# morriscb/chomp

Hardware: AMD Instinct MI355X
Metric: halo-model P(k,z) samples/sec (Stage K set-up + Stage E grid) (higher is better)
Workload: dtype f64

## Files before the change

### chomp_amd/csrc/chomp_mass_kernels.h

```cpp
#pragma once

#include <type_traits>

#include <hip/hip_runtime.h>

#include "../../include/chomp_mi355x.h"
#include "chomp_math.h"
#include "chomp_romberg.h"

namespace chomp {

enum { F_HM = 0, F_PPMM = 1, F_HG = 2, F_PPGM = 3, F_PPGG = 4, F_I12 = 5 };
constexpr int kFamilies = 6;

struct TabLayout {
  int NM, NK;
  int off_ln_mass, off_nu, off_nu_pp, off_lnm_pp;
  int off_knot[6], off_kpp[6];
  int off_levels, off_hf_lns2, off_misc;
  int stride;
  unsigned long long* h_status;
  unsigned h_seq;
};

inline TabLayout make_layout(int NM, int NK) {
  TabLayout L;
  L.NM = NM;
  L.NK = NK;
  int o = 0;
  L.off_ln_mass = o; o += NM;
  L.off_nu = o; o += NM;
  L.off_nu_pp = o; o += 4 * (NM - 1);
  L.off_lnm_pp = o; o += 4 * (NM - 1);
  for (int f = 0; f < kFamilies; ++f) { L.off_knot[f] = o; o += NK; }
  for (int f = 0; f < kFamilies; ++f) { L.off_kpp[f] = o; o += 4 * (NK - 1); }
  L.off_levels = o; o += kFamilies * NK;
  L.off_hf_lns2 = o; o += NK;
  L.off_misc = o; o += 8;
  L.stride = (o + 7) & ~7;
  L.h_status = nullptr;
  L.h_seq = 0u;
  return L;
}

constexpr int kNodeLevel = 10;
constexpr int kNodeTabLevel = 11;
constexpr int kNodeBase = (1 << kNodeLevel) + 1;
constexpr int kNodeCount = (1 << kNodeTabLevel) + 1;
constexpr int kNodeFields = 9;
constexpr int kNodeStride = kNodeFields * kNodeCount + 8;
__host__ __device__ inline int node_index(int lev, long j) {
  return lev == 0 ? (int)j : 1 + (1 << (lev - 1)) + (int)j;
}
typedef const double __attribute__((address_space(1)))* UniformDoubles;
__device__ __forceinline__ UniformDoubles uniform_ptr(const double* p) {
  const unsigned long long v = (unsigned long long)p;
  const unsigned lo = __builtin_amdgcn_readfirstlane((unsigned)v);
  const unsigned hi = __builtin_amdgcn_readfirstlane((unsigned)(v >> 32));
  return (UniformDoubles)(((unsigned long long)hi << 32) | lo);
}

constexpr int kKnotScratch = romberg_scratch<4, 2>();
constexpr int kSearchJ = 2048;
constexpr int kEpochDoubles = (int)(sizeof(Epoch) / sizeof(double));
static_assert(sizeof(Epoch) % sizeof(double) == 0, "Epoch must be 8-byte granular");

__device__ __forceinline__ bool same_cosmology(const Epoch& a, const Epoch& b) {
  return a.om0 == b.om0 && a.ob0 == b.ob0 && a.ol0 == b.ol0 && a.or0 == b.or0 &&
         a.tcmb == b.tcmb && a.h == b.h && a.ns == b.ns;
}

constexpr unsigned kStMassMinSaturated = CHOMP_ST_MASS_MIN_SATURATED;
constexpr unsigned kStMassMaxSaturated = CHOMP_ST_MASS_MAX_SATURATED;
constexpr unsigned kStSearchExhausted = CHOMP_ST_MASS_SEARCH_EXHAUSTED;
constexpr unsigned kStSigmaDivmax = CHOMP_ST_SIGMA_DIVMAX;
constexpr unsigned kStHaloDivmax0 = CHOMP_ST_HALO_DIVMAX_H_M;
constexpr unsigned kStNonfinite = CHOMP_ST_NONFINITE;
constexpr unsigned kStHaloBits = (63u * CHOMP_ST_HALO_DIVMAX_H_M) | CHOMP_ST_NONFINITE;

__device__ __forceinline__ void copy_doubles(double* dst, const double* src, int n) {
  for (int i = threadIdx.x; i < n; i += blockDim.x) dst[i] = src[i];
}

constexpr int kSigmaLevel = 13;
constexpr int kSigmaCount = (1 << kSigmaLevel) + 1;
constexpr int kSGrid = 48;
struct SGrid {
  double b0, b1, b2, b3, b4;
  bool valid;
  __host__ __device__ void segment(double x, double* lo, double* hi, int* n, int* off) const {
    if (x <= b1) { *lo = b0; *hi = b1; *n = 8; *off = 0; }
    else if (x <= b2) { *lo = b1; *hi = b2; *n = 14; *off = 8; }
    else if (x <= b3) { *lo = b2; *hi = b3; *n = 18; *off = 22; }
    else { *lo = b3; *hi = b4; *n = 8; *off = 40; }
  }
  __host__ __device__ double ln_r(int i) const {
    double lo, hi;
    int n, off;
    if (i < 8) { lo = b0; hi = b1; n = 8; off = 0; }
    else if (i < 22) { lo = b1; hi = b2; n = 14; off = 8; }
    else if (i < 40) { lo = b2; hi = b3; n = 18; off = 22; }
    else { lo = b3; hi = b4; n = 8; off = 40; }
    return lo + (hi - lo) * (double)(i - off) / (double)(n - 1);
  }
};
__host__ __device__ inline SGrid make_sgrid(double k_min, double k_max) {
  SGrid g;
  const double a = log(14.0662 / k_max) - log(100.0), b = log(14.0662 / k_max),
               c = log(0.1 / k_min);
  g.b0 = a - log(20.0);
  g.b1 = a; g.b2 = b; g.b3 = c;
  g.b4 = c + log(3.0);
  g.valid = b < c;
  return g;
}
constexpr int kSigmaOffI8 = 2 * kSigmaCount, kSigmaOffLnS = 2 * kSigmaCount + 8;
constexpr int kSigmaNodeBlocks = (kSigmaCount + 255) / 256;
constexpr int kSigmaOffPart = kSigmaOffLnS + kSGrid;
constexpr int kSigmaOffG = kSigmaOffPart + kSigmaNodeBlocks * (kSigmaLevel + 1);
constexpr int kGTabN = 8192;
constexpr int kGTabPad = 3;
static_assert(kGTabN == kGTabIntervals, "chomp_math.h: epoch_k_range");
constexpr int kGTabCount = kGTabN + 1 + 2 * kGTabPad;
constexpr int kGTabBlocks = (kGTabCount + 255) / 256;
constexpr int kSigmaStride = kSigmaOffG + 2 * kGTabCount;

struct SigmaInterpIntegrand {
  UniformDoubles g;
  double xlo, dx, inv_dx;
  double scale, amp2_nine_over_r6, amp2;
  bool tiny_r;
  SinCosLead lead = sincos_lead();
  __device__ __forceinline__ double operator()(double ln_k) const {
    const double u = (ln_k - xlo) * inv_dx;
    int i = (int)u;
    i = i < 0 ? 0 : (i > kGTabN - 1 ? kGTabN - 1 : i);
    const double t = u - (double)i;
    UniformDoubles q = g + i + kGTabPad - 2;
    const double a = t + 2.0, b = t + 1.0, d = t - 1.0, e = t - 2.0, f = t - 3.0;
    const double ab = a * b, ef = e * f, cd = t * d;
    const double gv = q[0] * (b * cd * ef) * (-1.0 / 120.0) + q[1] * (a * cd * ef) * (1.0 / 24.0) +
                      q[2] * (ab * d * ef) * (-1.0 / 12.0) + q[3] * (ab * t * ef) * (1.0 / 12.0) +
                      q[4] * (ab * cd * f) * (-1.0 / 24.0) + q[5] * (ab * cd * e) * (1.0 / 120.0);
    const double y = t * dx;
    const double ey = fma(y, fma(y, fma(y, fma(y, 1.0 / 24.0, 1.0 / 6.0), 0.5), 1.0), 1.0);
    const double k = q[2 + kGTabCount] * ey;
    const double kR = scale * k;
    if (tiny_r) {
      double s, c;
      fast_sincos_pm(kR, &s, &c);
      const double kR2 = kR * kR, k3 = k * k * k;
      const double W = 3.0 * (s / (kR2 * kR) - c / kR2);
      return amp2 * (gv * (k3 * k3)) * (W * W);
    }
    const double w = tophat_numer_pm(kR, lead);
    return amp2_nine_over_r6 * gv * (w * w);
  }
};

template <bool BAO>
__device__ __forceinline__ void sigma8_from_parts(const chomp_config& cfg, const Epoch& E,
                                                  double* __restrict__ n, int nb, double* red) {
  const double a = log(cfg.k_min), b = log(cfg.k_max);
  const bool tab8 = 0.1 / 8.0 > cfg.k_min && 14.0662 / 8.0 < cfg.k_max && cfg.divmax >= 1;
  __shared__ double stage[kSigmaNodeBlocks * (kSigmaLevel + 1)];
  __shared__ double S[kSigmaLevel + 1];
  __shared__ double i8;
  __shared__ int converged;
  for (int q = threadIdx.x; q < nb * (kSigmaLevel + 1); q += blockDim.x)
    stage[q] = __hip_atomic_load(n + kSigmaOffPart + q, __ATOMIC_RELAXED, __HIP_MEMORY_SCOPE_AGENT);
  __syncthreads();
  if (threadIdx.x <= kSigmaLevel) {
    double t = 0.0;
    for (int q = 0; q < nb; ++q) t += stage[q * (kSigmaLevel + 1) + threadIdx.x];
    S[threadIdx.x] = t;
  }
  __syncthreads();
  if (threadIdx.x < 64) {
    const int lane = threadIdx.x;
    const double range = b - a;
    double ordsum = 0.5 * S[0], nn = 1.0;
    double result = range * ordsum, prev = result;
    double Tl = lane == 0 ? result : 0.0;
    int conv = 0;
    const int top = cfg.divmax < kSigmaLevel ? cfg.divmax : kSigmaLevel;
    double crow[kSigmaLevel + 1];
#pragma unroll
    for (int i = 1; i <= kSigmaLevel; ++i) crow[i] = CHOMP_ROMBERG_C[i][lane & 31];
#pragma unroll
    for (int i = 1; i <= kSigmaLevel; ++i) {
      if (tab8 && i <= top && !conv) {
        nn *= 2.0;
        ordsum += S[i];
        const double Ti = ldexp(range * ordsum, -i);
        if (lane == i) Tl = Ti;
        result = wave_sum32(crow[i] * Tl);
        const double err = fabs(result - prev);
        prev = result;
        if (err < cfg.global_precision || err < cfg.cosmo_precision * fabs(result)) conv = 1;
      }
    }
    if (tab8 && !conv && cfg.divmax <= kSigmaLevel) conv = 1;
    if (lane == 0) {
      converged = conv;
      i8 = result;
    }
  }
  __syncthreads();
  if (!converged) {
    double lo, hi;
    sigma_limits(E, 8.0, &lo, &hi);
    SigmaIntegrandT<BAO> f{&E, 8.0};
    double s2;
    if (blockDim.x == 256) {
      s2 = romberg1<4>(f, lo, hi, cfg.global_precision, cfg.cosmo_precision, cfg.divmax, red);
    } else {
      s2 = 0.0;
      if (threadIdx.x < 64)
        s2 = romberg1<1>(f, lo, hi, cfg.global_precision, cfg.cosmo_precision, cfg.divmax, nullptr);
    }
    if (threadIdx.x == 0) i8 = s2;
  }
  if (threadIdx.x == 0) n[kSigmaOffI8] = i8;
}

template <int NPT>
__host__ __device__ constexpr int sigma_node_blocks() { return (kSigmaCount + 256 * NPT - 1) / (256 * NPT); }
template <int NPT>
__host__ __device__ constexpr int sigma_lns_blocks() { return NPT == 1 ? kSGrid : 0; }
template <int NPT>
__host__ __device__ constexpr int sigma_gtab_blocks() { return (kGTabCount + 256 * NPT - 1) / (256 * NPT); }

constexpr int kProbes = 4;
constexpr int kProbeStride = 24;
constexpr int kProbeLargeBatch = 128;

__host__ __device__ constexpr int sigma_epoch_rows(int n_epoch) { return (n_epoch + 255) / 256; }
__host__ __device__ constexpr int sigma_chi_rows(int n_epoch, int blocks_x) {
  return (n_epoch + blocks_x - 1) / blocks_x;
}

template <bool BAO, int NPT>
__global__ __launch_bounds__(256) void k_sigma_nodes(chomp_config cfg,
                                                     const chomp_cosmo* __restrict__ cosmo,
                                                     const double* __restrict__ zin,
                                                     const int* __restrict__ first,
                                                     const int* __restrict__ slots, int n_slots,
                                                     int n_epoch, Epoch* __restrict__ epochs,
                                                     double* __restrict__ snodes,
                                                     unsigned* __restrict__ status,
                                                     double* __restrict__ probe) {
  static_assert(NPT == 1 || NPT == 4, "nodes per thread");
  static_assert(kSGrid % 4 == 0, "four ln S points to a block");
  __shared__ Epoch E;
  __shared__ double red[romberg_scratch<4, 1>()];
  if ((int)blockIdx.y >= n_slots + sigma_epoch_rows(n_epoch)) {
    const int e = ((int)blockIdx.y - n_slots - sigma_epoch_rows(n_epoch)) * (int)gridDim.x +
                  (int)blockIdx.x;
    if (e >= n_epoch) return;
    const chomp_cosmo c = cosmo[e];
    const double z = zin[e] < 0.0 ? 0.0 : zin[e];
    EIntegrand f{c.omega_m0, c.omega_l0, c.omega_r0, 100.0 / (2.998 * 100000.0)};
    const double chi = romberg1<4>(f, 0.0, z, cfg.global_precision, cfg.cosmo_precision,
                                   cfg.divmax, red);
    if (threadIdx.x == 0) probe[(size_t)e * kProbeStride + 2 * kProbes] = chi;
    return;
  }
  if ((int)blockIdx.y >= n_slots) {
    const int e = ((int)blockIdx.y - n_slots) * 256 + (int)threadIdx.x;
    if (blockIdx.x != 0 || e >= n_epoch) return;
    Epoch B;
    double* q = reinterpret_cast<double*>(&B);
    for (int i = 0; i < kEpochDoubles; ++i) q[i] = 0.0;
    const chomp_cosmo c = cosmo[e];
    B.om0 = c.omega_m0; B.ob0 = c.omega_b0; B.ol0 = c.omega_l0; B.or0 = c.omega_r0;
    B.tcmb = c.cmb_temp; B.h = c.h; B.sigma8 = c.sigma_8; B.ns = c.n_scalar;
    B.z = zin[e];
    epoch_background(B, cfg.cosmo_precision, cfg.k_min, cfg.k_max, BAO ? 1 : 0);
    B.cosmo_slot = slots[e];
    epochs[e] = B;
    status[e] = 0u;
    return;
  }
  const int slot = blockIdx.y, e = first[slot];
  constexpr int nb = sigma_node_blocks<NPT>();
  constexpr int nl = sigma_lns_blocks<NPT>();
  if (threadIdx.x == 0) {
    const chomp_cosmo c = cosmo[e];
    E.om0 = c.omega_m0; E.ob0 = c.omega_b0; E.ol0 = c.omega_l0; E.or0 = c.omega_r0;
    E.tcmb = c.cmb_temp; E.h = c.h; E.sigma8 = c.sigma_8; E.ns = c.n_scalar;
    E.z = zin[e];
    epoch_shape_only(E, cfg.k_min, cfg.k_max, BAO ? 1 : 0);
  }
  __syncthreads();
  double* n = snodes + (size_t)slot * kSigmaStride;
  if ((int)blockIdx.x >= nb + nl) {
    const double xlo = log(cfg.k_min / 100.0), xhi = log(cfg.k_max * 100.0);
#pragma unroll
    for (int r = 0; r < NPT; ++r) {
      const int i = (((int)blockIdx.x - nb - nl) * NPT + r) * 256 + (int)threadIdx.x;
      if (i < kGTabCount) {
        const double x = xlo + (xhi - xlo) * ((double)(i - kGTabPad) / (double)kGTabN);
        const double k = exp(x);
        const double T = transfer_t<BAO>(E, k);
        const double k3 = k * k * k;
        n[kSigmaOffG + i] = exp((3.0 + E.ns) * (x - E.ln_H0)) * T * T / (k3 * k3);
        n[kSigmaOffG + kGTabCount + i] = k;
      }
    }
    return;
  }
  if ((int)blockIdx.x >= nb) {
    const int i = (int)blockIdx.x - nb;
    const double R = exp(make_sgrid(cfg.k_min, cfg.k_max).ln_r(i));
    double lo, hi;
    sigma_limits(E, R, &lo, &hi);
    SigmaIntegrandT<BAO> f{&E, R};
    const double s2 = romberg1<4>(f, lo, hi, cfg.global_precision, 1e-5,
                                  cfg.divmax < 10 ? cfg.divmax : 10, red);
    if (threadIdx.x == 0) n[kSigmaOffLnS + i] = log(s2);
    return;
  }
  const double a = log(cfg.k_min), b = log(cfg.k_max);
  const bool tab8 = 0.1 / 8.0 > cfg.k_min && 14.0662 / 8.0 < cfg.k_max && cfg.divmax >= 1;
  __shared__ double wsum[4][kSigmaLevel + 1];
  __shared__ int last_block;
  const int wv = threadIdx.x >> 6;
  if ((threadIdx.x & 63) <= kSigmaLevel) wsum[wv][threadIdx.x & 63] = 0.0;
#pragma unroll
  for (int r = 0; r < NPT; ++r) {
    const int first_idx = ((int)blockIdx.x * NPT + r) * 256;
    const int idx = first_idx + (int)threadIdx.x;
    const bool live = idx < kSigmaCount;
    int lev = 0;
    double g = 0.0;
    if (live) {
      double x;
      if (idx < 2) {
        x = idx == 0 ? a : b;
      } else {
        const int m = idx - 1;
        lev = 32 - __builtin_clz((unsigned)m);
        const long j = m - (1 << (lev - 1));
        const double h = ldexp(b - a, 1 - lev);
        x = (a + 0.5 * h) + h * (double)j;
      }
      const double k = exp(x);
      const double T = transfer_t<BAO>(E, k);
      n[idx] = k;
      const double k3 = k * k * k;
      const double d2k6 = exp((3.0 + E.ns) * (x - E.ln_H0)) * T * T / (k3 * k3);
      n[kSigmaCount + idx] = d2k6;
      const double t = tophat_numer_pm(8.0 * k);
      g = d2k6 * (9.0 / 262144.0) * (t * t);
    }
    if (first_idx < kSigmaCount) {
      const int last_idx = first_idx + 255;
      const int lev_lo = first_idx < 2 ? 0 : 32 - __builtin_clz((unsigned)(first_idx - 1));
      const int lev_hi = last_idx < 2 ? 0 : 32 - __builtin_clz((unsigned)(last_idx - 1));
      for (int l = lev_lo; l <= lev_hi && l <= kSigmaLevel; ++l) {
        const double v = wave_sum(live && lev == l ? g : 0.0);
        if ((threadIdx.x & 63) == 0) wsum[wv][l] += v;
      }
    }
  }
  double* part = n + kSigmaOffPart + (size_t)blockIdx.x * (kSigmaLevel + 1);
  __syncthreads();
  if (threadIdx.x <= kSigmaLevel) {
    __hip_atomic_store(part + threadIdx.x,
                       ((wsum[0][threadIdx.x] + wsum[1][threadIdx.x]) + wsum[2][threadIdx.x]) +
                           wsum[3][threadIdx.x],
                       __ATOMIC_RELAXED, __HIP_MEMORY_SCOPE_AGENT);
    asm volatile("s_waitcnt vmcnt(0)" ::: "memory");
  }
  if constexpr (NPT != 1) {
    return;
  } else {
    int* arrivals = reinterpret_cast<int*>(n + kSigmaOffI8 + 1);
    __syncthreads();
    if (threadIdx.x == 0) last_block = atomicAdd(arrivals, 1) == nb - 1 ? 1 : 0;
    __syncthreads();
    if (!last_block) return;
    if (threadIdx.x == 0) *arrivals = 0;
    sigma8_from_parts<BAO>(cfg, E, n, nb, red);
  }
}

struct SigmaInterpLds {
  static constexpr bool kLaneMajor = true;
  static constexpr bool kGeometric = true;
  const double* g;
  double xlo, dx, inv_dx, scale, nine_over_r6;
  bool tiny_r;
  SinCosLead lead = sincos_lead();
  __device__ __forceinline__ double operator()(double ln_k) const { return with_exp(ln_k, exp(ln_k)); }
  __device__ __forceinline__ double with_exp(double ln_k, double k) const {
    const double u = (ln_k - xlo) * inv_dx;
    int i = (int)u;
    i = i < 0 ? 0 : (i > kGTabN - 1 ? kGTabN - 1 : i);
    const double t = u - (double)i;
    const double* q = g + i + kGTabPad - 2;
    const double a = t + 2.0, b = t + 1.0, d = t - 1.0, e = t - 2.0, f = t - 3.0;
    const double ab = a * b, ef = e * f, cd = t * d;
    const double gv = q[0] * (b * cd * ef) * (-1.0 / 120.0) + q[1] * (a * cd * ef) * (1.0 / 24.0) +
                      q[2] * (ab * d * ef) * (-1.0 / 12.0) + q[3] * (ab * t * ef) * (1.0 / 12.0) +
                      q[4] * (ab * cd * f) * (-1.0 / 24.0) + q[5] * (ab * cd * e) * (1.0 / 120.0);
    const double kR = scale * k;
    if (tiny_r) {
      double s, c;
      fast_sincos_pm(kR, &s, &c);
      const double kR2 = kR * kR, k3 = k * k * k;
      const double W = 3.0 * (s / (kR2 * kR) - c / kR2);
      return (gv * (k3 * k3)) * (W * W);
    }
    const double w = tophat_numer_pm(kR, lead);
    return nine_over_r6 * gv * (w * w);
  }
};

constexpr int kLnsThreads = 512;
template <bool BAO>
__global__ __launch_bounds__(kLnsThreads) void k_sigma_lns(chomp_config cfg,
                                                           const chomp_cosmo* __restrict__ cosmo,
                                                           const double* __restrict__ zin,
                                                           const int* __restrict__ first,
                                                           double* __restrict__ snodes) {
  extern __shared__ __align__(16) double gl[];
  __shared__ Epoch E;
  const int slot = blockIdx.x, e = first[slot];
  double* n = snodes + (size_t)slot * kSigmaStride;
  if (threadIdx.x == 0) {
    const chomp_cosmo c = cosmo[e];
    E.om0 = c.omega_m0; E.ob0 = c.omega_b0; E.ol0 = c.omega_l0; E.or0 = c.omega_r0;
    E.tcmb = c.cmb_temp; E.h = c.h; E.sigma8 = c.sigma_8; E.ns = c.n_scalar;
    E.z = zin[e];
    epoch_shape_only(E, cfg.k_min, cfg.k_max, BAO ? 1 : 0);
  }
  if constexpr (!BAO) copy_doubles(gl, n + kSigmaOffG, kGTabCount);
  __syncthreads();
  sigma8_from_parts<BAO>(cfg, E, n, sigma_node_blocks<4>(), nullptr);
  __syncthreads();
  const SGrid G = make_sgrid(cfg.k_min, cfg.k_max);
  const double xlo = log(cfg.k_min / 100.0), xhi = log(cfg.k_max * 100.0);
  const double dx = (xhi - xlo) / (double)kGTabN;
  const int dmax = cfg.divmax < 10 ? cfg.divmax : 10;
  for (int i = (int)(threadIdx.x >> 6); i < kSGrid; i += kLnsThreads / 64) {
    const double R = exp(G.ln_r(i));
    double lo, hi;
    sigma_limits(E, R, &lo, &hi);
    double s2;
    if constexpr (BAO) {
      SigmaIntegrandT<BAO> f{&E, R};
      s2 = romberg1<1>(f, lo, hi, cfg.global_precision, 1e-5, dmax, nullptr);
    } else {
      const double r3 = R * R * R;
      SigmaInterpLds f{gl, xlo, dx, 1.0 / dx, R, 9.0 / (r3 * r3), 100.0 * E.k_max * R < 1.0};
      if (dmax >= 6) {
        Scalar1<SigmaInterpLds> w{f};
        static_assert(detail::lane_major<Scalar1<SigmaInterpLds>>::value, "lane-major level loop");
        const double fb[1] = {f(hi)};
        s2 = romberg_wave6<1>(w, lo, hi, fb, cfg.global_precision, 1e-5, dmax).value[0];
      } else {
        s2 = romberg1<1>(f, lo, hi, cfg.global_precision, 1e-5, dmax, nullptr);
      }
    }
    if ((threadIdx.x & 63) == 0) n[kSigmaOffLnS + i] = log(s2);
  }
}

template <bool BAO>
struct SigmaTabIntegrand {
  const Epoch* e;
  UniformDoubles node;
  UniformDoubles node_g;
  double scale, inv_amp;
  double nine_over_r6;
  SigmaInterpIntegrand deep;
  __device__ __forceinline__ void operator()(double ln_k, double (&out)[1], int lev,
                                             long j) const {
    if (lev <= kSigmaLevel) {
      const unsigned idx = (unsigned)node_index(lev, j) & 0x3fffu;
      const double kR = scale * node[idx];
      const double t = tophat_numer_pm(kR, deep.lead);
      out[0] = node_g[idx] * nine_over_r6 * (t * t);
    } else if (BAO) {
      SigmaIntegrandT<BAO> f{e, scale};
      out[0] = f(ln_k) * inv_amp;
    } else {
      out[0] = deep(ln_k);
    }
  }
};

template <int NW, int UNROLL = 1, bool BAO = false>
__device__ __forceinline__ double sigma2_block(const Epoch& E, const double* snode, double R,
                                               const chomp_config& cfg, double rtol,
                                               double* red, bool* converged = nullptr,
                                               const RombergLoose* loose = nullptr,
                                               int* level_out = nullptr) {
  const double need_min = 1.0 / R / 10.0, need_max = 1.0 / R * 14.0662;
  const double amp2 = E.amp * E.sigma_norm * E.sigma_norm;
  if (need_min > E.k_min && need_max < E.k_max) {
    const double lo = E.ln_k_min, hi = E.ln_k_max;
    const double r3 = R * R * R;
    const double nine_r6 = 9.0 / (r3 * r3);
    SigmaTabIntegrand<BAO> f{&E, uniform_ptr(snode), uniform_ptr(snode + kSigmaCount), R, 1.0 / amp2,
                             nine_r6,
                             SigmaInterpIntegrand{uniform_ptr(snode + kSigmaOffG), E.gtab_xlo, E.gtab_dx,
                                                  E.gtab_inv_dx, R, nine_r6, 1.0, false}};
    RombergLoose ls{0.0, 0.0, 0.0, 0.0, 0.0};
    if (loose) ls = RombergLoose{loose->rtol, loose->lo1 / amp2, loose->hi1 / amp2,
                                 loose->lo2 / amp2, loose->hi2 / amp2};
    RombergOut<1> r;
    bool fused = false;
    if constexpr (NW == 1) fused = cfg.divmax >= 6;
    if (fused) {
      double fb[1];
      f(hi, fb, 0, 1);
      r = romberg_wave6<1>(f, lo, hi, fb, cfg.global_precision, rtol, cfg.divmax, nullptr,
                           loose ? &ls : nullptr);
    } else {
      r = romberg_group<NW, 1, SigmaTabIntegrand<BAO>, UNROLL>(
          f, lo, hi, cfg.global_precision, rtol, cfg.divmax, red, nullptr, loose ? &ls : nullptr);
    }
    if (converged) *converged = r.converged[0];
    if (level_out) *level_out = r.level[0];
    return amp2 * r.value[0];
  }
  double lo, hi;
  sigma_limits(E, R, &lo, &hi);
  if constexpr (!BAO) {
    const double r3 = R * R * R;
    SigmaInterpIntegrand f{uniform_ptr(snode + kSigmaOffG), E.gtab_xlo, E.gtab_dx, E.gtab_inv_dx, R,
                           amp2 * 9.0 / (r3 * r3), amp2, 100.0 * E.k_max * R < 1.0};
    Scalar1<SigmaInterpIntegrand> w{f};
    RombergOut<1> r;
    bool fused = false;
    if constexpr (NW == 1) fused = cfg.divmax >= 6;
    if (fused) {
      const double fb[1] = {f(hi)};
      r = romberg_wave6<1>(w, lo, hi, fb, cfg.global_precision, rtol, cfg.divmax, nullptr, loose);
    } else {
      r = romberg_group<NW, 1>(w, lo, hi, cfg.global_precision, rtol, cfg.divmax, red, nullptr, loose);
    }
    if (converged) *converged = r.converged[0];
    if (level_out) *level_out = 100 + r.level[0];
    return r.value[0];
  } else {
    SigmaIntegrandT<BAO> f{&E, R};
    Scalar1<SigmaIntegrandT<BAO>> w{f};
    const RombergOut<1> r = romberg_group<NW, 1>(w, lo, hi, cfg.global_precision, rtol, cfg.divmax, red,
                                                 nullptr, loose);
    if (converged) *converged = r.converged[0];
    return r.value[0];
  }
}

__device__ __forceinline__ void spline_build_pcr(const double* x, const double* y, int n,
                                                 double* c, double* w, int tid, int tps,
                                                 bool active) {
  double *a0 = w, *b0 = w + n, *c0 = w + 2 * n, *d0 = w + 3 * n;
  double *a1 = w + 4 * n, *b1 = w + 5 * n, *c1 = w + 6 * n, *d1 = w + 7 * n;
  double* sl = w + 8 * n;
  if (active)
    for (int i = tid; i < n; i += tps) spline_row(x, y, n, i, &a0[i], &b0[i], &c0[i], &d0[i]);
  __syncthreads();
  for (int s = 1; s < n; s *= 2) {
    if (active)
      for (int i = tid; i < n; i += tps) pcr_step(n, i, s, a0, b0, c0, d0, a1, b1, c1, d1);
    __syncthreads();
    double* t;
    t = a0; a0 = a1; a1 = t;
    t = b0; b0 = b1; b1 = t;
    t = c0; c0 = c1; c1 = t;
    t = d0; d0 = d1; d1 = t;
  }
  if (active)
    for (int i = tid; i < n; i += tps) sl[i] = d0[i] / b0[i];
  __syncthreads();
  if (active)
    for (int i = tid; i < n - 1; i += tps) spline_coef(x, y, sl, i, c);
  __syncthreads();
}

template <int NW, int UNROLL = 1, bool BAO = false>
__device__ __forceinline__ double nu_of_mass_block(const Epoch& E, const double* snode,
                                                   double mass, const chomp_config& cfg,
                                                   double rtol, double* red,
                                                   bool* converged = nullptr,
                                                   const RombergLoose* loose = nullptr,
                                                   int* level_out = nullptr) {
  const double s2 = sigma2_block<NW, UNROLL, BAO>(E, snode, scale_of_mass(E, mass), cfg, rtol, red,
                                                  converged, loose, level_out);
  const double sq = E.delta_c / sqrt(s2);
  return sq * sq;
}

constexpr int kInitNW = 4;

struct SideThresholds {
  double thr_lo, thr_hi;
  const double *down, *up;
};
__device__ __forceinline__ SideThresholds side_thresholds(int side, const double* cand) {
  SideThresholds t;
  t.thr_lo = (side == 0 ? 0.1 : 50.0) * (1.0 - 0.05);
  t.thr_hi = (side == 0 ? 0.1 : 50.0) * (1.0 + 0.05);
  t.down = cand + (side == 0 ? 0 : 3) * kSearchJ;
  t.up = cand + (side == 0 ? 1 : 2) * kSearchJ;
  return t;
}

template <int NW, bool BAO>
__device__ __noinline__ double nu_probe(const Epoch& E, const double* snode, double m,
                                           const chomp_config& cfg, double thr_lo,
                                           double thr_hi, double* red) {
  const double kAmbiguous = 2e-5;
  const double rtol_probe = 1e-6;
  if (!(cfg.cosmo_precision < rtol_probe))
    return nu_of_mass_block<NW, 1, BAO>(E, snode, m, cfg, cfg.cosmo_precision, red);
  const double d2 = E.delta_c * E.delta_c;
  const double up = 1.0 + kAmbiguous, dn = 1.0 - kAmbiguous;
  const RombergLoose loose{rtol_probe, d2 / thr_hi * dn, d2 / thr_hi * up, d2 / thr_lo * dn,
                           d2 / thr_lo * up};
  return nu_of_mass_block<NW, 2, BAO>(E, snode, m, cfg, cfg.cosmo_precision, red, nullptr, &loose);
}

template <int NW, bool BAO>
__device__ double search_side_exact(const Epoch& E, const double* snode, int side,
                                    const chomp_config& cfg, const double* cand, double* red,
                                    int* n_eval, bool* exhausted, int seed_dir = 0,
                                    int seed_jl = 0, double nu_l = 0.0, int seed_jh = -1,
                                    double nu_h = 0.0) {
  const SideThresholds T = side_thresholds(side, cand);
  double mass = T.down[0];
  int dir = seed_dir;
  double nu0 = nu_l;
  if (seed_dir == 0) {
    nu0 = nu_probe<NW, BAO>(E, snode, T.down[0], cfg, T.thr_lo, T.thr_hi, red);
    ++*n_eval;
    if (T.thr_hi < nu0) dir = -1; else if (T.thr_lo > nu0) dir = +1;
  }
  if (dir != 0) {
    const double* tab = dir < 0 ? T.down : T.up;
    const double thr = dir < 0 ? T.thr_hi : T.thr_lo;
    int jl = seed_dir == 0 ? 0 : seed_jl, jh = seed_dir == 0 ? -1 : seed_jh;
    double tl = dir < 0 ? log(nu0 / thr) : log(thr / nu0);
    double th = jh < 0 ? 0.0 : (dir < 0 ? log(nu_h / thr) : log(thr / nu_h));
    double d = (side == 0 ? 0.25 : 0.7) * 0.04879;
    for (int it = 0; it < 4 * kSearchJ; ++it) {
      int jp;
      if (jh < 0) {
        double want = ceil(tl / d);
        if (!(want >= 1.0)) want = 1.0;
        if (want > 256.0) want = 256.0;
        jp = jl + (int)want;
        if (jp > kSearchJ - 1) jp = kSearchJ - 1;
      } else {
        if (jh == jl + 1) break;
        const double dd = (tl - th) / (double)(jh - jl);
        double want = ceil(tl / dd);
        if (!(want >= 1.0)) want = 1.0;
        if (want > (double)(jh - jl - 1)) want = (double)(jh - jl - 1);
        jp = jl + (int)want;
      }
      const double nu = nu_probe<NW, BAO>(E, snode, tab[jp], cfg, T.thr_lo, T.thr_hi, red);
      ++*n_eval;
      const bool pred = dir < 0 ? !(thr < nu) : !(thr > nu);
      const double tp = dir < 0 ? log(nu / thr) : log(thr / nu);
      if (pred) {
        jh = jp;
        th = tp;
      } else {
        if (jh < 0) {
          const double dn = (tl - tp) / (double)(jp - jl);
          d = dn > 1e-6 ? dn : 1e-6;
        }
        jl = jp;
        tl = tp;
        if (jh < 0 && jp == kSearchJ - 1) { jh = jp; *exhausted = true; break; }
      }
    }
    if (jh < 0) jh = jl;
    mass = tab[jh];
  }
  return mass;
}

__device__ __forceinline__ unsigned search_status(const Epoch& E, int side, double mass,
                                                  bool exhausted) {
  const double R = scale_of_mass(E, mass);
  unsigned st = 0u;
  if (side == 0 && 100.0 * E.k_max * R < 0.2) st |= kStMassMinSaturated;
  if (side == 1 && 0.1 / R <= E.k_min / 100.0) st |= kStMassMaxSaturated;
  if (exhausted) st |= kStSearchExhausted;
  return st;
}

__device__ __forceinline__ double ln_s_estimate(const SGrid& G, const double* lns, double x) {
  if (!G.valid || !(x >= G.b0 && x <= G.b4)) return NAN;
  double lo, hi;
  int n, off;
  G.segment(x, &lo, &hi, &n, &off);
  const double u = (x - lo) / (hi - lo) * (double)(n - 1);
  int i0 = (int)floor(u) - 2;
  i0 = i0 < 0 ? 0 : (i0 > n - 6 ? n - 6 : i0);
  const double* f = lns + off + i0;
  const double t = u - (double)i0;
  const double t0 = t, t1 = t - 1.0, t2 = t - 2.0, t3 = t - 3.0, t4 = t - 4.0, t5 = t - 5.0;
  return f[0] * (t1 * t2 * t3 * t4 * t5) * (-1.0 / 120.0) +
         f[1] * (t0 * t2 * t3 * t4 * t5) * (1.0 / 24.0) +
         f[2] * (t0 * t1 * t3 * t4 * t5) * (-1.0 / 12.0) +
         f[3] * (t0 * t1 * t2 * t4 * t5) * (1.0 / 12.0) +
         f[4] * (t0 * t1 * t2 * t3 * t5) * (-1.0 / 24.0) +
         f[5] * (t0 * t1 * t2 * t3 * t4) * (1.0 / 120.0);
}

struct SidePlan {
  bool ok;
  int dir, j;
  double nu_start;
  bool at_edge;
};
__device__ __forceinline__ SidePlan plan_side(const Epoch& E, const double* lns, int side,
                                              const double* cand, int* sh) {
  const SideThresholds T = side_thresholds(side, cand);
  const SGrid G = make_sgrid(E.k_min, E.k_max);
  const double margin = 1e-2;
  const double ln_margin = 0.00995033085;
  SidePlan P{false, 0, 0, 0.0, false};
  const int lane = threadIdx.x & 63;
  const double arg = lane == 0 ? E.delta_c * E.delta_c / (E.amp * E.sigma_norm * E.sigma_norm)
                   : lane == 1 ? 3.0 * T.down[0] / (4.0 * kPi * E.rho_bar)
                   : lane == 2 ? T.thr_hi : T.thr_lo;
  const double lg = log(arg);
  const double ln_nu_c = readlane_d(lg, 0), x0 = readlane_d(lg, 1) * (1.0 / 3.0);
  const double ln_hi = readlane_d(lg, 2), ln_lo = readlane_d(lg, 3);
  const double step = 0.016263388 ;
  const double ln_nu0 = ln_nu_c - ln_s_estimate(G, lns, x0);
  P.nu_start = exp(ln_nu0);
  if (!(ln_nu0 == ln_nu0)) return P;
  if (ln_nu0 > ln_hi + ln_margin) P.dir = -1;
  else if (ln_nu0 < ln_lo - ln_margin) P.dir = +1;
  else if (ln_nu0 >= ln_lo + ln_margin && ln_nu0 <= ln_hi - ln_margin) {
    P.ok = true;
    return P;
  } else {
    P.ok = true;
    P.at_edge = true;
    P.dir = P.nu_start > 0.5 * (T.thr_lo + T.thr_hi) ? -1 : +1;
    P.j = 2;
    return P;
  }
  (void)margin;
  const double ln_thr = P.dir < 0 ? ln_hi : ln_lo;
  auto passes = [&](int j) {
    const double ln_nu = ln_nu_c - ln_s_estimate(G, lns, x0 + (double)(P.dir * j) * step);
    return !(ln_nu == ln_nu) || (P.dir < 0 ? !(ln_thr < ln_nu) : !(ln_thr > ln_nu));
  };
  constexpr int kStride = kSearchJ / 256;
  __syncthreads();
  if (threadIdx.x == 0) *sh = kSearchJ;
  __syncthreads();
  for (int t = (int)threadIdx.x; t < 256; t += (int)blockDim.x) {
    const int j = kStride * (1 + t) - 1;
    if (j < kSearchJ && passes(j)) atomicMin(sh, j);
  }
  __syncthreads();
  const int jc = *sh;
  __syncthreads();
  if (jc < kSearchJ && (int)threadIdx.x < kStride - 1) {
    const int j = jc - (kStride - 1) + (int)threadIdx.x;
    if (j >= 1 && passes(j)) atomicMin(sh, j);
  }
  __syncthreads();
  const int j = *sh;
  if (j >= kSearchJ) return P;
  const double lsj = ln_s_estimate(G, lns, x0 + (double)(P.dir * j) * step);
  if (!(lsj == lsj)) return P;
  P.j = j;
  P.ok = true;
  return P;
}

template <class F>
decltype(auto) with_flag(bool flag, F&& f) {
  return flag ? f(std::true_type{}) : f(std::false_type{});
}
template <class F>
decltype(auto) with_flag(bool a, bool b, F&& f) {
  return with_flag(a, [&](auto A) { return with_flag(b, [&](auto B) { return f(A, B); }); });
}
template <int N>
using int_c = std::integral_constant<int, N>;

void launch_epoch_probe(bool bao, unsigned n_epoch, hipStream_t stream, const chomp_config& cfg,
                        Epoch* epochs, double* search, const double* cand, const double* snodes,
                        double* probe, int* count, unsigned* status);

template <bool BAO, int NW, bool SIG = false>
__global__ __launch_bounds__(64 * NW) void k_nu_table(chomp_config cfg, TabLayout L,
                                                      const Epoch* __restrict__ epochs,
                                                      const double* __restrict__ search,
                                                      const double* __restrict__ snodes,
                                                      double* __restrict__ tab,
                                                      unsigned* __restrict__ status,
                                                      int epochs_fastest,
                                                      double* __restrict__ sig = nullptr,
                                                      int sig_stride = 0) {
  __shared__ Epoch E;
  __shared__ double red[romberg_scratch<NW, 1>()];
  int e = epochs_fastest ? (int)blockIdx.x : (int)blockIdx.y;
  int i = (int)blockIdx.x;
  if (!epochs_fastest) {
    const int NM = (int)gridDim.x, n = (int)gridDim.y;
    const int b = (int)blockIdx.x + NM * (int)blockIdx.y;
    if (b < 8 * NM * (n / 8)) {
      const int slot = b >> 3;
      e = (slot / NM) * 8 + (b & 7);
      i = slot % NM;
    }
  }
  if (epochs_fastest) {
    const int NM = (int)gridDim.y, y = (int)blockIdx.y, m0 = NM / 2 - 1;
    if (NM < 8) i = NM - 1 - y;
    else if (y < 2) i = m0 + y;
    else if (y >= NM - 2) i = m0 + 2 + (y - (NM - 2));
    else { i = NM - 1 - (y - 2); if (i <= m0 + 3) i -= 4; }
  }
  copy_doubles(reinterpret_cast<double*>(&E), reinterpret_cast<const double*>(&epochs[e]),
               kEpochDoubles);
  __syncthreads();
  const double* snode = snodes + (size_t)E.cosmo_slot * kSigmaStride;
  const double ln_lo = search[(e * 2 + 0) * 2], ln_hi = search[(e * 2 + 1) * 2];
  const double lnm = linspace_at(ln_lo, ln_hi, L.NM, i);
  bool conv = true;
  double nu;
  if constexpr (SIG) {
    const double s2 = sigma2_block<NW, 1, BAO>(E, snode, scale_of_mass(E, exp(lnm)), cfg,
                                               cfg.cosmo_precision, red, &conv);
    const double sq = E.delta_c / sqrt(s2);
    nu = sq * sq;
    if (threadIdx.x == 0) sig[(size_t)e * sig_stride + i] = sqrt(s2);
  } else {
    nu = nu_of_mass_block<NW, 1, BAO>(E, snode, exp(lnm), cfg, cfg.cosmo_precision, red, &conv);
  }
  if (threadIdx.x == 0) {
    double* t = tab + (size_t)e * L.stride;
    t[L.off_ln_mass + i] = lnm;
    t[L.off_nu + i] = nu;
    if (!conv) atomicOr(&status[e], kStSigmaDivmax);
  }
}

struct TinkerTab {
  double x[9];
  double c[5][32];
};

struct FnuLn {
  const Epoch* e;
  __device__ __forceinline__ double operator()(double t) const {
    const double nu = exp(t);
    return f_nu(*e, nu) * nu;
  }
};
struct FnuLin {
  const Epoch* e;
  __device__ __forceinline__ double operator()(double nu) const { return f_nu(*e, nu); }
};
struct FnuBiasLin {
  const Epoch* e;
  __device__ __forceinline__ double operator()(double nu) const {
    return f_nu(*e, nu) * bias_nu(*e, nu);
  }
};
constexpr int kNormLiteralDivmax = 18;
struct FnuBiasLn {
  const Epoch* e;
  __device__ __forceinline__ double operator()(double t) const {
    const double nu = exp(t);
    return f_nu(*e, nu) * bias_nu(*e, nu) * nu;
  }
};

struct MassLds {
  double *x_lnm, *y_nu, *c_nu, *c_lnm, *work, *gl, *red;
  __device__ __forceinline__ void carve(double* sm, int NM) {
    x_lnm = sm;
    y_nu = x_lnm + NM;
    c_nu = y_nu + NM;
    c_lnm = c_nu + 4 * (NM - 1);
    work = c_lnm + 4 * (NM - 1);
    gl = work + 18 * NM;
    red = gl + 32;
  }
};
__host__ __device__ inline int mass_lds_doubles(int NM) {
  return 2 * NM + 8 * (NM - 1) + 18 * NM + 32 + romberg_scratch<4, 2>();
}

template <class Beside>
__device__ __forceinline__ void mass_setup_block(
    const chomp_config& cfg, const TabLayout& L, Epoch& E, Epoch* __restrict__ epochs, int e,
    bool publish, double ln_mass_min, double ln_mass_max, int n_search, double* __restrict__ t,
    const chomp_halo_par& hp, int mf_kind, const TinkerTab* __restrict__ tinker,
    const double* __restrict__ gl16, const MassLds& M, Beside&& beside) {
  const int NM = L.NM;
  copy_doubles(M.x_lnm, t + L.off_ln_mass, NM);
  copy_doubles(M.y_nu, t + L.off_nu, NM);
  copy_doubles(M.gl, gl16, 32);
  __syncthreads();
  {
    const int sys = threadIdx.x >> 7, tid = threadIdx.x & 127;
    spline_build_pcr(sys == 0 ? M.x_lnm : M.y_nu, sys == 0 ? M.y_nu : M.x_lnm, NM,
                     sys == 0 ? M.c_nu : M.c_lnm, M.work + sys * 9 * NM, tid, 128, true);
  }
  if (threadIdx.x < 64) {
    const int lane = (int)threadIdx.x;
    const double mf_delta_v = (hp.delta_v == -1.0) ? E.delta_v : hp.delta_v;
    double mine = 0.0;
    if (mf_kind == CHOMP_MF_TINKER && lane < 5) {
      const double ld = log(mf_delta_v);
      const double opz = 1.0 + E.z;
      mine = spline_eval(tinker->x, tinker->c[lane], 9, ld);
      const double ex = lane == 1 ? 0.20 : (lane == 2 ? -0.01 : (lane == 3 ? -0.08 : 0.27));
      if (lane > 0) mine *= pow(opz, ex);
    }
    if (lane == 5) mine = exp(spline_eval(M.y_nu, M.c_lnm, NM, 1.0));
    const double t_alpha = readlane_d(mine, 0), t_beta = readlane_d(mine, 1);
    const double t_gamma = readlane_d(mine, 2), t_phi = readlane_d(mine, 3);
    const double t_eta = readlane_d(mine, 4), m_star = readlane_d(mine, 5);
    if (lane == 0) {
      E.ln_mass_min = ln_mass_min;
      E.ln_mass_max = ln_mass_max;
      E.n_search = n_search;
      E.nu_min = 1.001 * M.y_nu[0];
      E.nu_max = 0.999 * M.y_nu[NM - 1];
      E.m_star = m_star;
      E.stq = hp.stq;
      E.st_a = hp.st_little_a;
      E.mf_delta_v = mf_delta_v;
      E.mf_kind = mf_kind;
      E.f_norm = 1.0;
      E.bias_norm = 1.0;
      E.ln_st_a = log(hp.st_little_a);
      E.ln_t_beta = 0.0;
      if (mf_kind == CHOMP_MF_TINKER) {
        E.t_alpha = t_alpha;
        E.t_beta = t_beta;
        E.t_gamma = t_gamma;
        E.t_phi = t_phi;
        E.t_eta = t_eta;
        E.ln_t_beta = log(E.t_beta);
        tinker_bias_constants(E);
      }
    }
  }
  __syncthreads();
  int flip = 0;
  const bool literal = cfg.divmax < kNormLiteralDivmax;
  const double a = log(E.nu_min), b = log(E.nu_max);
  if (literal) {
    if (mf_kind == CHOMP_MF_ST) {
      FnuLin f{&E};
      const double norm = romberg1<4>(f, E.nu_min, E.nu_max, cfg.global_precision,
                                      cfg.mass_precision, cfg.divmax, M.red);
      __syncthreads();
      if (threadIdx.x == 0) E.f_norm = 1.0 / norm;
      __syncthreads();
    }
    FnuBiasLin f{&E};
    const double norm = romberg1<4>(f, E.nu_min, E.nu_max, cfg.global_precision,
                                    cfg.mass_precision, cfg.divmax, M.red);
    __syncthreads();
    if (threadIdx.x == 0) E.bias_norm = 1.0 / norm;
    if (threadIdx.x >= blockDim.x - 64) beside();
    __syncthreads();
  } else {
    constexpr int NT = 256;
    const double wd = (b - a) / 8.0;
    double p1 = 0.0, p2 = 0.0;
    if (threadIdx.x >= NT - 64) beside();
    for (int idx = threadIdx.x; idx < 16 * 8; idx += NT) {
      const int pn = idx >> 4, q = idx & 15;
      const double mid = a + wd * ((double)pn + 0.5);
      const double nu = exp(mid + 0.5 * wd * M.gl[q]);
      const double fn = f_nu(E, nu) * nu;
      p1 += M.gl[16 + q] * fn;
      p2 += M.gl[16 + q] * (fn * bias_nu(E, nu));
    }
    const double i1 = 0.5 * wd * group_sum<4>(p1, M.red, flip);
    const double i2 = 0.5 * wd * group_sum<4>(p2, M.red, flip);
    __syncthreads();
    if (threadIdx.x == 0) {
      const double fnorm = mf_kind == CHOMP_MF_ST ? 1.0 / i1 : 1.0;
      E.f_norm = fnorm;
      E.bias_norm = 1.0 / (fnorm * i2);
    }
    __syncthreads();
  }
  if (!publish) return;
  copy_doubles(reinterpret_cast<double*>(&epochs[e]), reinterpret_cast<const double*>(&E),
               kEpochDoubles);
  copy_doubles(t + L.off_nu_pp, M.c_nu, 4 * (NM - 1));
  copy_doubles(t + L.off_lnm_pp, M.c_lnm, 4 * (NM - 1));
}

}
```

Measured before the change: 2.324 billion.

## Replace adaptive Romberg for ln-sigma grid with single-pass fixed-level sum; add inverse crossing search

The per-radius sigma integral used to run an adaptive Romberg loop capped at ten levels. It is replaced by a single pass that evaluates all points of the finest level at once, forms the trapezoid sums for every level from wave reductions, and combines them with precomputed Romberg coefficients. This removes the iterative convergence loop and its synchronisations, at the cost of always evaluating the full point set and dropping the early-exit tolerance. Separately, plan_side first estimates the threshold-crossing index by root-finding on the tabulated ln-sigma grid. It then verifies that guess with two probes and falls back to the block-wide atomic search only when the check fails.

Result: faster. 2.355 billion (median of 6 runs) (+1.3%).

```diff
diff --git a/chomp_amd/csrc/chomp_mass_kernels.h b/chomp_amd/csrc/chomp_mass_kernels.h
--- a/chomp_amd/csrc/chomp_mass_kernels.h
+++ b/chomp_amd/csrc/chomp_mass_kernels.h
@@ -224,6 +224,53 @@
   if (threadIdx.x == 0) n[kSigmaOffI8] = i8;
 }
 
+constexpr int kLnsLevel = 10;
+template <class F>
+__device__ __forceinline__ double lns_one_pass(const F& f, double a, double b, int L) {
+  static_assert(kLnsLevel == 10, "four points per thread of 256");
+  __shared__ double lsum[4][kLnsLevel + 1];
+  __shared__ double ends[2];
+  const int lane = threadIdx.x & 63, wv = threadIdx.x >> 6;
+  const int N = 1 << L;
+  const double range = b - a;
+  const double crow = CHOMP_ROMBERG_C[L][lane & 31];
+  double v[4];
+#pragma unroll
+  for (int r = 0; r < 4; ++r) {
+    const int p = (int)threadIdx.x + 256 * r;
+    v[r] = p < N ? f(a + ldexp(range * (double)p, -L)) : 0.0;
+  }
+  if (threadIdx.x == 255) ends[1] = f(b);
+  if (threadIdx.x == 0) {
+    ends[0] = v[0];
+    v[0] = 0.0;
+  }
+  if (lane <= kLnsLevel) lsum[wv][lane] = 0.0;
+  const double mine = (v[0] + v[1]) + (v[2] + v[3]);
+  const int tz = lane == 0 ? -1 : __builtin_ctz((unsigned)lane);
+#pragma unroll
+  for (int c = 0; c < 6; ++c) {
+    const double s = wave_sum(tz == c ? mine : 0.0);
+    if (lane == 0 && L - c >= 1) lsum[wv][L - c] = s;
+  }
+  if (lane == 0) {
+#pragma unroll
+    for (int r = 0; r < 4; ++r) {
+      const int p = (int)threadIdx.x + 256 * r;
+      if (p > 0 && p < N) lsum[wv][L - __builtin_ctz((unsigned)p)] += v[r];
+    }
+  }
+  __syncthreads();
+  double T = 0.0;
+  if (lane <= L) {
+    double ordsum = 0.5 * (ends[0] + ends[1]);
+    for (int l = 1; l <= lane; ++l)
+      ordsum += ((lsum[0][l] + lsum[1][l]) + lsum[2][l]) + lsum[3][l];
+    T = ldexp(range * ordsum, -lane);
+  }
+  return wave_sum32(crow * T);
+}
+
 template <int NPT>
 __host__ __device__ constexpr int sigma_node_blocks() { return (kSigmaCount + 256 * NPT - 1) / (256 * NPT); }
 template <int NPT>
@@ -316,8 +363,7 @@
     double lo, hi;
     sigma_limits(E, R, &lo, &hi);
     SigmaIntegrandT<BAO> f{&E, R};
-    const double s2 = romberg1<4>(f, lo, hi, cfg.global_precision, 1e-5,
-                                  cfg.divmax < 10 ? cfg.divmax : 10, red);
+    const double s2 = lns_one_pass(f, lo, hi, cfg.divmax < kLnsLevel ? cfg.divmax : kLnsLevel);
     if (threadIdx.x == 0) n[kSigmaOffLnS + i] = log(s2);
     return;
   }
@@ -721,14 +767,41 @@
   int dir, j;
   double nu_start;
   bool at_edge;
-};
+  bool searched;
+};
+
+__device__ __forceinline__ double crossing_index(const SGrid& G, const double* lns, double x0,
+                                                 int dir, double step, double target) {
+  if (!G.valid) return NAN;
+  const int lane = threadIdx.x & 63;
+  bool brackets = false;
+  if (lane < kSGrid - 1 && lane != 7 && lane != 21 && lane != 39) {
+    const double xl = G.ln_r(lane), xr = G.ln_r(lane + 1);
+    brackets = lns[lane] >= target && lns[lane + 1] < target && (dir < 0 ? xl < x0 : xr > x0);
+  }
+  const unsigned long long m = __ballot(brackets);
+  if (m == 0ull) return NAN;
+  const int ib = dir < 0 ? 63 - __builtin_clzll(m) : __builtin_ctzll(m);
+  double xa = G.ln_r(ib), xb = G.ln_r(ib + 1);
+  double ga = lns[ib] - target, gb = lns[ib + 1] - target;
+  const double x1 = xa + (xb - xa) * (ga / (ga - gb));
+  const double g1 = ln_s_estimate(G, lns, x1) - target;
+  if (g1 >= 0.0) { xa = x1; ga = g1; } else { xb = x1; gb = g1; }
+  const double x2 = xa + (xb - xa) * (ga / (ga - gb));
+  const double g2 = ln_s_estimate(G, lns, x2) - target;
+  double x3 = x2;
+  if (g2 != g1) x3 = x2 - g2 * ((x2 - x1) / (g2 - g1));
+  return (x3 - x0) / ((double)dir * step);
+}
+
+template <bool INVERSE = true>
 __device__ __forceinline__ SidePlan plan_side(const Epoch& E, const double* lns, int side,
                                               const double* cand, int* sh) {
   const SideThresholds T = side_thresholds(side, cand);
   const SGrid G = make_sgrid(E.k_min, E.k_max);
   const double margin = 1e-2;
   const double ln_margin = 0.00995033085;
-  SidePlan P{false, 0, 0, 0.0, false};
+  SidePlan P{false, 0, 0, 0.0, false, false};
   const int lane = threadIdx.x & 63;
   const double arg = lane == 0 ? E.delta_c * E.delta_c / (E.amp * E.sigma_norm * E.sigma_norm)
                    : lane == 1 ? 3.0 * T.down[0] / (4.0 * kPi * E.rho_bar)
@@ -758,6 +831,21 @@
     const double ln_nu = ln_nu_c - ln_s_estimate(G, lns, x0 + (double)(P.dir * j) * step);
     return !(ln_nu == ln_nu) || (P.dir < 0 ? !(ln_thr < ln_nu) : !(ln_thr > ln_nu));
   };
+  if constexpr (INVERSE) {
+    const double jr = ceil(crossing_index(G, lns, x0, P.dir, step, ln_nu_c - ln_thr));
+    if (jr >= 1.0 && jr <= (double)(kSearchJ - 1)) {
+      const int j = (int)jr;
+      const double lsj = ln_s_estimate(G, lns, x0 + (double)(P.dir * j) * step);
+      const double ln_nu = ln_nu_c - lsj;
+      const bool pass_j = lsj == lsj && (P.dir < 0 ? !(ln_thr < ln_nu) : !(ln_thr > ln_nu));
+      if (pass_j && (j == 1 || !passes(j - 1))) {
+        P.j = j;
+        P.ok = true;
+        return P;
+      }
+    }
+  }
+  P.searched = true;
   constexpr int kStride = kSearchJ / 256;
   __syncthreads();
   if (threadIdx.x == 0) *sh = kSearchJ;
```
